# gau-nernst/vision-toolbox

Measured on AMD Instinct MI355X. Metric: images/sec (node) CSPDarknet-53 bf16 train step @224px, higher is better.
Workload: dtype bf16; 1 GPU; cspdarknet53 train step (fwd+CE+bwd+allreduce+SGD), batch 256/GPU, 3x224x224, 1000 classes, BASELINE configs[1]; global_batch=256, per_gpu_batch=256, parallelism=dp1, rccl_ranks=1, local_device=cuda:0, hip_graphs=False, main_stream_priority=-1, sync_bn=False, deterministic=False

## Files before the change

vision-toolbox_amd/csrc/vt_igemm.hip:

```cpp
#include <stdlib.h>

#include "vt_common.h"
#include "vt_igemm_args.h"

namespace {

constexpr int kTapBytes = VT_MAX_TAPS * 16;
constexpr int stat_bytes(int WM, int BN) { return WM * 2 * BN * 4 > 2048 ? WM * 2 * BN * 4 : 2048; }

__device__ __attribute__((aligned(16))) unsigned int vt_zero16[4];

__device__ __forceinline__ int swz(int row) { return (0x1320 >> (((row >> 2) & 3) * 4)) & 3; }

__device__ __forceinline__ void glds16(const void* gsrc, unsigned lds_base) {
    unsigned keep;
    asm volatile(
        "s_mov_b32 %0, m0\n\t"
        "s_mov_b32 m0, %2\n\t"
        "s_nop 0\n\t"
        "global_load_lds_dwordx4 %1, off\n\t"
        "s_mov_b32 m0, %0"
        : "=&s"(keep)
        : "v"(gsrc), "s"(lds_base)
        : "memory");
}

template <int N>
__device__ __forceinline__ void vm_wait() {
    asm volatile("s_waitcnt vmcnt(%0)" ::"n"(N) : "memory");
}

template <typename T>
__device__ __forceinline__ void mma(const uint4& a, const uint4& b, f32x4& acc);

template <>
__device__ __forceinline__ void mma<bf16_t>(const uint4& a, const uint4& b, f32x4& acc) {
    acc = __builtin_amdgcn_mfma_f32_16x16x32_bf16(__builtin_bit_cast(bf16x8, a),
                                                  __builtin_bit_cast(bf16x8, b), acc, 0, 0, 0);
}
template <>
__device__ __forceinline__ void mma<float>(const uint4& a, const uint4& b, f32x4& acc) {
    acc = __builtin_amdgcn_mfma_f32_16x16x4f32(__uint_as_float(a.x), __uint_as_float(b.x), acc, 0, 0, 0);
    acc = __builtin_amdgcn_mfma_f32_16x16x4f32(__uint_as_float(a.y), __uint_as_float(b.y), acc, 0, 0, 0);
    acc = __builtin_amdgcn_mfma_f32_16x16x4f32(__uint_as_float(a.z), __uint_as_float(b.z), acc, 0, 0, 0);
    acc = __builtin_amdgcn_mfma_f32_16x16x4f32(__uint_as_float(a.w), __uint_as_float(b.w), acc, 0, 0, 0);
}

template <int BM, int BN, int PD, int NW, int WM>
struct Geom {
    static constexpr int NI_A = BM / 16;
    static constexpr int NI = (BM + BN) / 16;
    static constexpr int IT = (NI + NW - 1) / NW;
    static constexpr int SS = IT * NW * 64;
    static constexpr int HDR = kTapBytes + stat_bytes(WM, BN);
    static constexpr int NS = PD + 1;
    static constexpr int STAGE_BYTES = NS * SS * 16;
};

template <typename T, int BM, int BN, int WM, int WN, int PD, bool UK>
__global__ void __launch_bounds__(64 * WM * WN) igemm_kernel(const IgemmArgs p) {
    constexpr int NW = WM * WN;
    using G = Geom<BM, BN, PD, NW, WM>;
    constexpr int NT = 64 * NW;
    constexpr int kHdrBytes = G::HDR;
    constexpr int EPC = 16 / sizeof(T);
    constexpr int BK = 4 * EPC;
    constexpr int TM = BM / WM, TN = BN / WN, FM = TM / 16, FN = TN / 16;
    constexpr int IT = G::IT, SS = G::SS, NS = G::NS;
    static_assert(NW == 4 || NW == 8, "4 or 8 waves per workgroup");
    static_assert(TM % 16 == 0 && TN % 16 == 0, "wave tile must be 16-granular");
    static_assert(BN <= 160, "filter tile width");
    static_assert(BM % 16 == 0 && BN % 16 == 0, "tile rows come in groups of 16 per DMA instruction");
    static_assert(PD >= 1 && PD <= 3, "prefetch distance");

    extern __shared__ __attribute__((aligned(16))) char smem[];
    int4* sTap = (int4*)smem;
    float* sStat = (float*)(smem + kTapBytes);
    uint4* sStage = (uint4*)(smem + kHdrBytes);
    T* sOut = (T*)(smem + kHdrBytes);

    const int tid = threadIdx.x;
    const int lane = tid & 63;
    const int wave = __builtin_amdgcn_readfirstlane(tid >> 6);
    const int wm = wave / WN, wn = wave % WN;

    const int bid = blockIdx.x;
    const int xcd = bid & 7, slot = bid >> 3;
    const int tn = slot % p.tiles_n;
    const int ml = slot / p.tiles_n;
    const int tm = xcd * p.chunk + ml;
    if (ml >= p.chunk || tm >= p.tiles_m) return;

#pragma unroll
    for (int t = 0; t < VT_MAX_TAPS; ++t) {
        if (t < p.ntaps && tid == t) {
            const int dh = p.dh[t], dw = p.dw[t];
            sTap[t] = make_int4(dh, dw, (dh * p.Wi + dw) * p.ldx, 0);
        }
    }
    if (tid < 2 * BN) sStat[tid] = 0.f;
    __syncthreads();

    const T* __restrict__ xg = (const T*)p.x;
    const T* __restrict__ wg = (const T*)p.w;
    const unsigned long zero_src = (unsigned long)(const void*)vt_zero16;
    const unsigned ring_base = (unsigned)(unsigned long)(__attribute__((address_space(3))) char*)sStage;

    const int cj = (lane & 3) ^ ((0x1320 >> (((lane >> 4) & 3) * 4)) & 3);
    int hb[IT], wb[IT];
    long off0[IT];
    bool valid[IT];
    const int HoWo = p.Ho * p.Wo;
#pragma unroll
    for (int i = 0; i < IT; ++i) {
        const int j = wave + NW * i;
        hb[i] = wb[i] = 0;
        off0[i] = 0;
        valid[i] = false;
        if (j < G::NI_A) {
            const int row = j * 16 + (lane >> 2);
            const int m = tm * BM + row;
            valid[i] = m < p.M;
            const int mm = valid[i] ? m : 0;
            const int b = mm / HoWo;
            const int rem = mm - b * HoWo;
            const int oi = rem / p.Wo;
            const int oj = rem - oi * p.Wo;
            hb[i] = oi * p.sh + p.h0;
            wb[i] = oj * p.sw + p.w0;
            off0[i] = ((long)(b * p.Hi + hb[i]) * p.Wi + wb[i]) * p.ldx;
        } else if (j < G::NI) {
            const int n = tn * BN + (j - G::NI_A) * 16 + (lane >> 2);
            valid[i] = n < p.Cout;
            off0[i] = (long)(valid[i] ? n : 0) * p.ldw;
        }
    }

    int kk = cj * EPC;
    int tap = kk / p.Cin;
    int c = kk - tap * p.Cin;

    unsigned long abase[IT], amask[IT], bptr[IT];
    unsigned bstep[IT];
    int tap_u = 0, c0_u = 0;
    if constexpr (UK) {
#pragma unroll
        for (int i = 0; i < IT; ++i) {
            const int j = wave + NW * i;
            abase[i] = (unsigned long)(xg + (off0[i] + cj * EPC));
            amask[i] = 0;
            bptr[i] = zero_src;
            bstep[i] = 0;
            if (j < G::NI_A) {
                if (valid[i]) {
                    for (int t = 0; t < p.ntaps; ++t) {
                        const int4 te = sTap[t];
                        if ((unsigned)(hb[i] + te.x) < (unsigned)p.Hi && (unsigned)(wb[i] + te.y) < (unsigned)p.Wi)
                            amask[i] |= 1ul << t;
                    }
                }
            } else if (j < G::NI && valid[i]) {
                bptr[i] = (unsigned long)(wg + (off0[i] + cj * EPC));
                bstep[i] = BK * (unsigned)sizeof(T);
            }
        }
    }

#define VT_ISSUE_STAGE(st)                                                                      \
    do {                                                                                        \
        if constexpr (UK) {                                                                     \
            const long koff = ((long)__builtin_amdgcn_readfirstlane(sTap[tap_u].z) + c0_u) * (long)sizeof(T); \
            _Pragma("unroll") for (int i = 0; i < IT; ++i) {                                    \
                const int j = wave + NW * i;                                                     \
                const bool isA = (NW * i + NW - 1 < G::NI_A) ? true : (NW * i >= G::NI_A ? false : j < G::NI_A); \
                unsigned long ps;                                                               \
                if (isA) {                                                                      \
                    ps = ((amask[i] >> tap_u) & 1ul) ? abase[i] + koff : zero_src;              \
                } else {                                                                        \
                    ps = bptr[i];                                                               \
                    bptr[i] += bstep[i];                                                        \
                }                                                                               \
                glds16((const void*)ps, ring_base + (unsigned)(((st)*SS + j * 64) * 16));       \
            }                                                                                   \
            c0_u += BK;                                                                         \
            if (c0_u >= p.Cin) {                                                                \
                c0_u = 0;                                                                       \
                ++tap_u;                                                                        \
            }                                                                                   \
            break;                                                                              \
        }                                                                                       \
        const bool kval = tap < p.ntaps;                                                        \
        const int4 te = sTap[kval ? tap : 0];                                                   \
        _Pragma("unroll") for (int i = 0; i < IT; ++i) {                                        \
            const int j = wave + NW * i;                                                         \
              \
            const bool isA = (NW * i + NW - 1 < G::NI_A) ? true : (NW * i >= G::NI_A ? false : j < G::NI_A); \
            const bool isB = !isA && ((NW * i + NW - 1 < G::NI) ? true : (NW * i >= G::NI ? false : j < G::NI)); \
            const bool va = kval && valid[i] && (unsigned)(hb[i] + te.x) < (unsigned)p.Hi &&    \
                            (unsigned)(wb[i] + te.y) < (unsigned)p.Wi;                          \
            const unsigned long pa = (unsigned long)(xg + (off0[i] + te.z + c));                \
            const unsigned long pb = (unsigned long)(wg + (off0[i] + kk));                      \
            const unsigned long ps = isA ? (va ? pa : zero_src) : ((isB && kval && valid[i]) ? pb : zero_src); \
            glds16((const void*)ps, ring_base + (unsigned)(((st)*SS + j * 64) * 16));           \
        }                                                                                       \
        kk += BK;                                                                               \
        c += BK;                                                                                \
        while (c >= p.Cin) {                                                                    \
            c -= p.Cin;                                                                         \
            ++tap;                                                                              \
        }                                                                                       \
    } while (0)

    f32x4 acc[FM][FN];
#pragma unroll
    for (int i = 0; i < FM; ++i)
#pragma unroll
        for (int j = 0; j < FN; ++j) acc[i][j] = f32x4{0.f, 0.f, 0.f, 0.f};

    const int lane_off = (lane & 15) * 4 + ((lane >> 4) ^ swz(lane & 15));
    const int nk = (p.Ktot + BK - 1) / BK;

#pragma unroll
    for (int s = 0; s < PD; ++s)
        if (s < nk) VT_ISSUE_STAGE(s);

    int cur = 0;
    int nxt = PD % NS;
    for (int ks = 0; ks < nk; ++ks) {
        const int younger = min(PD - 1, nk - 1 - ks);
        if (younger >= 2)
            vm_wait<2 * IT>();
        else if (younger == 1)
            vm_wait<IT>();
        else
            vm_wait<0>();
        __builtin_amdgcn_s_barrier();
        asm volatile("" ::: "memory");
        if (ks + PD < nk) VT_ISSUE_STAGE(nxt);
        {
            const uint4* A = sStage + cur * SS + wm * TM * 4 + lane_off;
            const uint4* Bt = sStage + cur * SS + BM * 4 + wn * TN * 4 + lane_off;
            uint4 af[FM], bf[FN];
#pragma unroll
            for (int i = 0; i < FM; ++i) af[i] = A[i * 64];
#pragma unroll
            for (int j = 0; j < FN; ++j) bf[j] = Bt[j * 64];
#if VT_MFMA_SETPRIO
            __builtin_amdgcn_s_setprio(1);
#endif
#pragma unroll
            for (int i = 0; i < FM; ++i)
#pragma unroll
                for (int j = 0; j < FN; ++j) mma<T>(af[i], bf[j], acc[i][j]);
#if VT_MFMA_SETPRIO
            __builtin_amdgcn_s_setprio(0);
#endif
        }
        cur = (cur + 1 == NS) ? 0 : cur + 1;
        nxt = (nxt + 1 == NS) ? 0 : nxt + 1;
    }
#undef VT_ISSUE_STAGE
    __syncthreads();

    const bool affine = p.flags & VT_CONV_AFFINE;
    const bool relu = p.flags & VT_CONV_RELU;
    const bool stats = p.flags & VT_CONV_STATS;
#pragma unroll
    for (int j = 0; j < FN; ++j) {
        const int col = wn * TN + j * 16 + (lane & 15);
        const int n = tn * BN + col;
        float sc = 1.f, sf = 0.f;
        if (affine && n < p.Cout) {
            if (p.scale) sc = p.scale[n];
            sf = p.shift[n];
        }
        float s = 0.f, ss = 0.f;
#pragma unroll
        for (int i = 0; i < FM; ++i) {
#pragma unroll
            for (int r = 0; r < 4; ++r) {
                float v = acc[i][j][r];
                if (affine) v = fmaf(v, sc, sf);
                if (relu) v = fmaxf(v, 0.f);
                const T tv = from_float<T>(v);
                const int row = wm * TM + i * 16 + (lane >> 4) * 4 + r;
                sOut[row * BN + col] = tv;
                const float fv = (float)tv;
                s += fv;
                ss += fv * fv;
            }
        }
        if (stats) {
            s += __shfl_xor(s, 16, 64);
            s += __shfl_xor(s, 32, 64);
            ss += __shfl_xor(ss, 16, 64);
            ss += __shfl_xor(ss, 32, 64);
            if (lane < 16) {
                sStat[(wm * 2 + 0) * BN + col] = s;
                sStat[(wm * 2 + 1) * BN + col] = ss;
            }
        }
    }
    __syncthreads();

    if (stats && tid < 2 * BN) {
        const int which = tid / BN, col = tid % BN;
        const int n = tn * BN + col;
        if (n < p.Cout) {
            float acc = 0.f;
#pragma unroll
            for (int w = 0; w < WM; ++w) acc += sStat[(w * 2 + which) * BN + col];
            vt_stat_add(p.stats, ((long)(tm % kStatReplicas) * 2 + which) * p.Cout + n, acc);
        }
    }

    constexpr int CPR = BN / EPC;
    const uint4* sOut4 = (const uint4*)sOut;
    T* __restrict__ yg = (T*)p.y;
    const T* __restrict__ rg = (const T*)p.res;
    const bool has_res = (p.flags & VT_CONV_RESIDUAL) != 0;
    auto out_pixel = [&](int m) -> long {
        if (p.dense_out) return m;
        const int b = m / HoWo;
        const int rem = m - b * HoWo;
        const int oi = rem / p.Wo;
        const int oj = rem - oi * p.Wo;
        return ((long)b * p.oH + (oi * p.oHs + p.oh0)) * p.oW + (oj * p.oWs + p.ow0);
    };
    if (has_res) {
        constexpr int ITER = (BM * CPR + NT - 1) / NT, RB = 4;
#pragma unroll
        for (int b0 = 0; b0 < ITER; b0 += RB) {
            uint4 rr[RB];
            long oy[RB];
            bool ok[RB];
#pragma unroll
            for (int u = 0; u < RB; ++u) {
                const int idx = tid + (b0 + u) * NT;
                const int row = idx / CPR, ch = idx % CPR;
                const int m = tm * BM + row;
                const int n = tn * BN + ch * EPC;
                ok[u] = b0 + u < ITER && idx < BM * CPR && m < p.M && n < p.Cout;
                const long po = ok[u] ? out_pixel(m) : 0;
                oy[u] = po * p.ldy + vt_out_col(p, n, p.ldy);
                rr[u] = *(const uint4*)(rg + (ok[u] ? po * p.ldr + vt_out_col(p, n, p.ldr) : 0l));
            }
#pragma unroll
            for (int u = 0; u < RB; ++u) {
                if (!ok[u]) continue;
                float fv[EPC], fr[EPC];
                VecIO<T>::unpack(sOut4[tid + (b0 + u) * NT], fv);
                VecIO<T>::unpack(rr[u], fr);
#pragma unroll
                for (int e = 0; e < EPC; ++e) fv[e] += fr[e];
                *(uint4*)(yg + oy[u]) = VecIO<T>::pack(fv);
            }
        }
        return;
    }
#pragma unroll 2
    for (int idx = tid; idx < BM * CPR; idx += NT) {
        const int row = idx / CPR, ch = idx % CPR;
        const int m = tm * BM + row;
        const int n = tn * BN + ch * EPC;
        if (m < p.M && n < p.Cout) *(uint4*)(yg + (out_pixel(m) * p.ldy + vt_out_col(p, n, p.ldy))) = sOut4[idx];
    }
}

template <typename T, int BM, int BN, int WM, int WN, int PD>
int launch(IgemmArgs& a, hipStream_t st) {
    using G = Geom<BM, BN, PD, WM * WN, WM>;
    constexpr int kHdrBytes = G::HDR;
    a.tiles_m = (a.M + BM - 1) / BM;
    a.tiles_n = (a.Cout + BN - 1) / BN;
    a.chunk = (a.tiles_m + 7) / 8;
    constexpr int outb = BM * BN * (int)sizeof(T);
    constexpr int smem = kHdrBytes + (G::STAGE_BYTES > outb ? G::STAGE_BYTES : outb);
    static_assert(smem <= 160 * 1024, "tile exceeds the 160 KiB LDS of a gfx950 CU");
    const long blocks = (long)8 * a.chunk * a.tiles_n;
    if (blocks > 0x7fffffffL) {
        vt_set_error("vt_conv_igemm: grid too large (%ld blocks)", blocks);
        return VT_ERR_UNSUPPORTED;
    }
    constexpr int BKe = 4 * (16 / (int)sizeof(T));
    auto kern = (a.Cin % BKe == 0) ? igemm_kernel<T, BM, BN, WM, WN, PD, true>
                                   : igemm_kernel<T, BM, BN, WM, WN, PD, false>;
    if (smem > 64 * 1024) {
        const int rc = vt_raise_dynamic_lds((const void*)kern, smem, "vt_conv_igemm");
        if (rc != VT_OK) return rc;
    }
    vt_note_kernel("igemm_kernel<%s,%d,%d,%d,%d,%d,uk%d>", sizeof(T) == 2 ? "bf16" : "f32", BM, BN, WM, WN, PD,
                   (int)(a.Cin % BKe == 0));
    hipLaunchKernelGGL(kern, dim3((unsigned)blocks), dim3(64 * WM * WN), smem, st, a);
    VT_CHECK_LAUNCH("vt_conv_igemm");
    return VT_OK;
}

}

static void fill_args(IgemmArgs& a, const vt_conv_desc* d, const void* x, const void* w, void* y, const float* scale,
                      const float* shift, const void* residual, float* stats) {
    memset(&a, 0, sizeof(a));
    a.x = x;
    a.w = w;
    a.y = y;
    a.scale = scale;
    a.shift = shift;
    a.res = residual;
    a.stats = stats;
    a.B = d->B, a.Hi = d->Hi, a.Wi = d->Wi, a.Cin = d->Cin, a.ldx = d->ldx;
    a.Ho = d->Ho, a.Wo = d->Wo, a.sh = d->sh, a.sw = d->sw, a.h0 = d->h0, a.w0 = d->w0;
    a.Cout = d->Cout, a.ldy = d->ldy, a.oH = d->oH, a.oW = d->oW;
    a.oHs = d->oHs, a.oWs = d->oWs, a.oh0 = d->oh0, a.ow0 = d->ow0;
    a.ldw = d->ldw, a.ldr = d->ldr, a.flags = d->flags, a.ntaps = d->ntaps;
    a.M = d->B * d->Ho * d->Wo;
    a.Ktot = d->ntaps * d->Cin;
    a.dense_out = (d->oHs == 1 && d->oWs == 1 && d->oh0 == 0 && d->ow0 == 0 && d->oH == d->Ho && d->oW == d->Wo);
    memcpy(a.dh, d->dh, VT_MAX_TAPS);
    memcpy(a.dw, d->dw, VT_MAX_TAPS);

}

extern "C" int vt_conv_igemm(const vt_conv_desc* d, const void* x, const void* w, void* y,
                             const float* scale, const float* shift, const void* residual,
                             float* stats, void* stream) {
    VT_REQUIRE(d && x && w && (y || (d->flags & VT_CONV_NOSTORE)), VT_ERR_INVALID, "vt_conv_igemm: null argument");
    VT_REQUIRE(!(d->flags & VT_CONV_NOSTORE) || (d->flags & VT_CONV_STATS), VT_ERR_INVALID,
               "vt_conv_igemm: NOSTORE is the statistics-only pass");
    VT_REQUIRE(d->dtype == VT_F32 || d->dtype == VT_BF16, VT_ERR_UNSUPPORTED,
               "vt_conv_igemm: dtype %d", d->dtype);
    VT_REQUIRE(!(d->flags & VT_CONV_BNRED), VT_ERR_INVALID, "vt_conv_igemm: unknown flag bits 0x%x", d->flags);
    const int epc = vt_epc(d->dtype);
    VT_REQUIRE(d->ntaps >= 1 && d->ntaps <= VT_MAX_TAPS, VT_ERR_UNSUPPORTED,
               "vt_conv_igemm: ntaps %d outside [1,%d]", d->ntaps, VT_MAX_TAPS);
    VT_REQUIRE(d->B > 0 && d->Hi > 0 && d->Wi > 0 && d->Ho > 0 && d->Wo > 0 && d->Cin > 0 && d->Cout > 0,
               VT_ERR_INVALID, "vt_conv_igemm: non-positive extent");
    VT_REQUIRE(d->Cin % epc == 0 && d->Cout % epc == 0 && d->ldx % epc == 0 && d->ldy % epc == 0 &&
                   d->ldw % epc == 0,
               VT_ERR_UNSUPPORTED,
               "vt_conv_igemm: Cin=%d Cout=%d ldx=%d ldy=%d ldw=%d must be multiples of %d", d->Cin,
               d->Cout, d->ldx, d->ldy, d->ldw, epc);
    const bool d2s = (d->flags & VT_CONV_D2S) != 0;
    if (d2s) {
        VT_REQUIRE(d->Cout % (4 * epc) == 0 && d->oHs == 2 && d->oWs == 2 && d->oh0 == 0 && d->ow0 == 0 &&
                       d->oH == 2 * d->Ho && d->oW == 2 * d->Wo &&
                       !(d->flags & (VT_CONV_STATS | VT_CONV_AFFINE | VT_CONV_RELU)),
                   VT_ERR_UNSUPPORTED, "vt_conv_igemm: D2S needs Cout = 4*C', a 2x2-strided output and a raw epilogue");
    }
    VT_REQUIRE(d->ldx >= d->Cin && d->ldy >= (d2s ? d->Cout / 4 : d->Cout) && d->ldw >= d->ntaps * d->Cin, VT_ERR_INVALID,
               "vt_conv_igemm: stride smaller than extent");
    VT_REQUIRE(vt_aligned16(x) && vt_aligned16(w) && vt_aligned16(y), VT_ERR_INVALID,
               "vt_conv_igemm: x/w/y must be 16-byte aligned");
    VT_REQUIRE(d->oHs >= 1 && d->oWs >= 1 && d->oh0 >= 0 && d->ow0 >= 0 &&
                   (d->Ho - 1) * d->oHs + d->oh0 < d->oH && (d->Wo - 1) * d->oWs + d->ow0 < d->oW,
               VT_ERR_INVALID, "vt_conv_igemm: output placement outside the %dx%d tensor", d->oH, d->oW);
    const long in_elems = (long)d->B * d->Hi * d->Wi * d->ldx;
    const long out_elems = (long)d->B * d->oH * d->oW * d->ldy;
    VT_REQUIRE(in_elems < 0x7fffffffL && out_elems < 0x7fffffffL && (long)d->B * d->Ho * d->Wo < 0x7fffffffL,
               VT_ERR_UNSUPPORTED, "vt_conv_igemm: tensor exceeds 2^31 elements");
    if (d->flags & VT_CONV_RESIDUAL) {
        VT_REQUIRE(residual && vt_aligned16(residual) && d->ldr % epc == 0 && d->ldr >= (d2s ? d->Cout / 4 : d->Cout),
                   VT_ERR_INVALID, "vt_conv_igemm: bad residual");
    }
    if (d->flags & VT_CONV_AFFINE) VT_REQUIRE(shift, VT_ERR_INVALID, "vt_conv_igemm: AFFINE needs shift");
    if (d->flags & VT_CONV_STATS) {
        VT_REQUIRE(stats, VT_ERR_INVALID, "vt_conv_igemm: STATS needs a stats buffer");
        VT_REQUIRE(!(d->flags & (VT_CONV_AFFINE | VT_CONV_RELU | VT_CONV_RESIDUAL)), VT_ERR_UNSUPPORTED,
                   "vt_conv_igemm: STATS is only defined on the raw conv output");
    }

    IgemmArgs a;
    fill_args(a, d, x, w, y, scale, shift, residual, stats);

    hipStream_t st = (hipStream_t)stream;
    if (!d2s) {
        const int rc = vt_stem_dispatch(a, d->dtype, stream);
        if (rc >= 0) return rc;
        const int rc6 = vt_stem6_dispatch(a, d->dtype, stream);
        if (rc6 >= 0) return rc6;
    }
    VT_REQUIRE(!(d->flags & VT_CONV_NOSTORE), VT_ERR_UNSUPPORTED, "vt_conv_igemm: NOSTORE outside the RGB stem kernel");
    if (!d2s) {
        const int rc = vt_span6_dispatch(a, d->dtype, stream);
        if (rc >= 0) return rc;
    }
    {
        const int rc = vt_pspan_dispatch(a, d->dtype, stream);
        if (rc >= 0) return rc;
    }
    {
        const int rc = vt_span_dispatch(a, d->dtype, stream);
        if (rc >= 0) return rc;
    }
    if (d->dtype == VT_BF16) {
        const int w8 = VT_KNOB("VT_IGEMM_W8", 3);
        if (VT_KNOB("VT_IGEMM_BN80", 1) && d->Cout % 80 == 0 && d->Cout <= 160) {
            if ((w8 & 1) && d->Cout == 160) return launch<bf16_t, 256, 160, 4, 2, 2>(a, st);
            return launch<bf16_t, 256, 80, 4, 1, 2>(a, st);
        }
        if (d->Cout > 64 && (w8 & 2) && ((long)(a.M + 255) / 256) * ((d->Cout + 127) / 128) >= ((w8 & 4) ? 0 : 256))
            return launch<bf16_t, 256, 128, 4, 2, 2>(a, st);
        if (d->Cout > 64) return launch<bf16_t, 128, 128, 2, 2, 2>(a, st);
        if (d->Cout > 32) return launch<bf16_t, 128, 64, 2, 2, 2>(a, st);
        return launch<bf16_t, 256, 32, 4, 1, 2>(a, st);
    }
    if (d->Cout > 32) return launch<float, 128, 64, 2, 2, 2>(a, st);
    return launch<float, 128, 32, 4, 1, 2>(a, st);
}

extern "C" int vt_conv_dgrad_bnred(const vt_conv_desc* d, const void* dz, const void* w, void* dy, const void* z, int32_t ldz,
                                   const float* scale, const float* shift, const float* mean, const float* invstd,
                                   int32_t relu, float* sums, void* stream) {
    VT_REQUIRE(d && dz && w && dy && z && scale && shift && mean && invstd && sums, VT_ERR_INVALID,
               "vt_conv_dgrad_bnred: null argument");
    VT_REQUIRE(relu == 0 || relu == 1, VT_ERR_UNSUPPORTED, "vt_conv_dgrad_bnred: activation code %d (none / ReLU only)", relu);
    VT_REQUIRE(d->flags == 0, VT_ERR_INVALID, "vt_conv_dgrad_bnred: the launch has a plain epilogue (flags 0x%x)", d->flags);
    const long M = (long)d->B * d->oH * d->oW;
    const bool whole = d->oHs == 1 && d->oWs == 1 && d->oh0 == 0 && d->ow0 == 0 && d->oH == d->Ho && d->oW == d->Wo;
    VT_REQUIRE(whole, VT_ERR_INVALID, "vt_conv_dgrad_bnred: the launch must produce every pixel of d(y)");
    const int epc = vt_epc(d->dtype);
    VT_REQUIRE(ldz % epc == 0 && ldz >= d->Cout && vt_aligned16(z), VT_ERR_INVALID, "vt_conv_dgrad_bnred: bad z");
    if (d->dtype == VT_BF16 && VT_KNOB("VT_DGRAD_BNRED", 1) && d->ntaps >= 1 && d->ntaps <= VT_MAX_TAPS && d->Cin % epc == 0 &&
        d->Cout % epc == 0 && d->ldx % epc == 0 && d->ldy % epc == 0 && d->ldw % epc == 0 && d->ldx >= d->Cin &&
        d->ldy >= d->Cout && d->ldw >= d->ntaps * d->Cin && vt_aligned16(dz) && vt_aligned16(w) && vt_aligned16(dy) &&
        (long)d->B * d->Hi * d->Wi * d->ldx < 0x7fffffffL && M * d->ldy < 0x7fffffffL && M * ldz < 0x7fffffffL) {
        IgemmArgs a;
        fill_args(a, d, dz, w, dy, scale, shift, z, sums);
        a.ldr = ldz;
        a.aux0 = mean, a.aux1 = invstd;
        a.flags = VT_CONV_BNRED | (relu ? VT_CONV_RELU : 0);
        const int rc = vt_span6_dispatch(a, d->dtype, stream);
        if (rc >= 0) return rc;
    }
    const int rc = vt_conv_igemm(d, dz, w, dy, nullptr, nullptr, nullptr, nullptr, stream);
    if (rc != VT_OK) return rc;
    return vt_bn_act_bwd_reduce(dy, d->ldy, z, ldz, scale, shift, mean, invstd, M, d->Cout, relu, d->dtype, sums, stream);
}
```

vision-toolbox_amd/csrc/vt_igemm_args.h:

```cpp
#pragma once
#include "vt_common.h"

#define VT_CONV_BNRED 0x1000

#ifndef VT_MFMA_SETPRIO
#define VT_MFMA_SETPRIO 0
#endif

struct IgemmArgs {
    const void* x;
    const void* w;
    void* y;
    const float* scale;
    const float* shift;
    const void* res;
    float* stats;
    int B, Hi, Wi, Cin, ldx, Ho, Wo, sh, sw, h0, w0, Cout, ldy, oH, oW, oHs, oWs, oh0, ow0;
    int ldw, ldr, flags, ntaps;
    int M, Ktot, tiles_m, tiles_n, chunk, dense_out;
    int fast_dma;
    int8_t dh[VT_MAX_TAPS];
    int8_t dw[VT_MAX_TAPS];
    const float* aux0;
    const float* aux1;
};

__device__ __forceinline__ long vt_out_col(const IgemmArgs& p, int n, int ld) {
    if (!(p.flags & VT_CONV_D2S)) return n;
    const int cq = p.Cout >> 2;
    const int blk = n / cq;
    return ((long)(blk >> 1) * p.oW + (blk & 1)) * ld + (n - blk * cq);
}

int vt_span_dispatch(IgemmArgs& a, int dtype, void* stream);

int vt_span6_dispatch(IgemmArgs& a, int dtype, void* stream);

int vt_pspan_dispatch(IgemmArgs& a, int dtype, void* stream);

int vt_stem_dispatch(IgemmArgs& a, int dtype, void* stream);

int vt_stem6_dispatch(IgemmArgs& a, int dtype, void* stream);
```

Baseline: 13220 images/sec.

## Add persistent weight-stationary 1x1 conv GEMM kernel with register ring prefetch

Adds a dedicated bf16 kernel for stride-1 1x1 convolutions. The kernel loads a full BN-column weight slab into LDS once per block. Waves then stream 32-row activation blocks through a 3–4 deep register ring feeding MFMA 16x16x32, with fused epilogue and optional fused BN statistics. It is dispatched ahead of the generic pspan/span paths, but only for a narrow M/Cin window, and by default only for the stats-producing case. The aim is to cut weight reloads and per-tile overhead of the generic implicit GEMM, at the cost of low occupancy and large LDS use.

```diff
diff --git a/vision-toolbox_amd/csrc/vt_gemm1x1.hip b/vision-toolbox_amd/csrc/vt_gemm1x1.hip
--- /dev/null
+++ b/vision-toolbox_amd/csrc/vt_gemm1x1.hip
@@ -0,0 +1,284 @@
+#include <type_traits>
+
+#include "vt_igemm_args.h"
+
+namespace {
+
+constexpr int kRows = 32;
+constexpr int kFM = kRows / 16;
+constexpr int kThreads = 512;
+
+struct G1Args {
+    IgemmArgs p;
+    int ksteps;
+    int nrb;
+    int gx, gy;
+};
+
+__device__ __forceinline__ float sum16(float x) {
+    x += __shfl_xor(x, 8, 64);
+    x += __shfl_xor(x, 4, 64);
+    x += __shfl_xor(x, 2, 64);
+    x += __shfl_xor(x, 1, 64);
+    return x;
+}
+
+template <int BN, bool STATS, int RS>
+__global__ __launch_bounds__(kThreads, 4) void gemm1x1_kernel(const G1Args a) {
+    constexpr int NF = BN / 16;
+    constexpr int NG = BN / 32;
+    extern __shared__ __attribute__((aligned(16))) char smem[];
+    const IgemmArgs& p = a.p;
+    const unsigned item = vt_xcd_item(blockIdx.x, gridDim.x, 8);
+    if (item >= (unsigned)(a.gx * a.gy)) return;
+    const int tn = (int)(item % (unsigned)a.gy), bx = (int)(item / (unsigned)a.gy);
+    const int n0 = tn * BN;
+    const int tid = threadIdx.x, lane = tid & 63;
+    const int wave = __builtin_amdgcn_readfirstlane(tid >> 6);
+    const int lrow = lane & 15, lq = lane >> 4;
+    const int KS = a.ksteps;
+
+    {
+        const bf16_t* __restrict__ wg = (const bf16_t*)p.w;
+        const int per_col = KS * 4;
+        for (int idx = tid; idx < BN * per_col; idx += kThreads) {
+            const int c = idx / per_col, rem = idx - c * per_col;
+            const int ks = rem >> 2, q4 = rem & 3;
+            uint4 v = make_uint4(0u, 0u, 0u, 0u);
+            if (n0 + c < p.Cout) v = *(const uint4*)(wg + ((long)(n0 + c) * p.ldw + ks * 32 + q4 * 8));
+            const int g = c >> 5, cc = c & 31;
+            const int f = 2 * g + ((cc >> 2) & 1), r = 4 * (cc >> 3) + (cc & 3);
+            *(uint4*)(smem + (((long)ks * NF + f) * 64 + (q4 * 16 + r)) * 16) = v;
+        }
+    }
+    __syncthreads();
+
+    const int stride = a.gx * (kThreads / 64);
+    const int first = bx * (kThreads / 64) + wave;
+    const bf16_t* __restrict__ xg = (const bf16_t*)p.x;
+    bf16_t* __restrict__ yg = (bf16_t*)p.y;
+    const bf16_t* rg = (const bf16_t*)p.res;
+    const bool has_res = (p.flags & VT_CONV_RESIDUAL) != 0;
+    const bool affine = (p.flags & VT_CONV_AFFINE) != 0;
+    const bool relu = (p.flags & VT_CONV_RELU) != 0;
+
+    float s1[STATS ? NG : 1][8], s2[STATS ? NG : 1][8];
+    if (STATS) {
+#pragma unroll
+        for (int g = 0; g < NG; ++g)
+#pragma unroll
+            for (int e = 0; e < 8; ++e) s1[g][e] = s2[g][e] = 0.f;
+    }
+
+    int rb_l = first, ks_l = 0;
+    const bf16_t* lp[kFM];
+    auto set_lp = [&]() __attribute__((always_inline)) {
+#pragma unroll
+        for (int i = 0; i < kFM; ++i) {
+            long m = (long)rb_l * kRows + i * 16 + lrow;
+            m = m < p.M ? m : (long)p.M - 1;
+            lp[i] = xg + (m * p.ldx + lq * 8);
+        }
+    };
+    set_lp();
+    uint4 ring[RS][kFM];
+#pragma unroll
+    for (int s = 0; s < RS; ++s)
+#pragma unroll
+        for (int i = 0; i < kFM; ++i) ring[s][i] = make_uint4(0u, 0u, 0u, 0u);
+    auto issue = [&](auto Sc) __attribute__((always_inline)) {
+        constexpr int S = decltype(Sc)::value;
+        if (rb_l < a.nrb) {
+#pragma unroll
+            for (int i = 0; i < kFM; ++i) ring[S][i] = *(const uint4*)(lp[i] + ks_l * 32);
+            if (++ks_l == KS) {
+                ks_l = 0;
+                rb_l += stride;
+                set_lp();
+            }
+        }
+    };
+
+    f32x4 acc[kFM][NF];
+    auto zero_acc = [&]() __attribute__((always_inline)) {
+#pragma unroll
+        for (int i = 0; i < kFM; ++i)
+#pragma unroll
+            for (int f = 0; f < NF; ++f) acc[i][f] = f32x4{0.f, 0.f, 0.f, 0.f};
+    };
+    zero_acc();
+
+    auto epilogue = [&](int rb) __attribute__((always_inline)) {
+#pragma unroll
+        for (int i = 0; i < kFM; ++i) {
+            const long m = (long)rb * kRows + i * 16 + lrow;
+            const bool row_ok = m < p.M;
+#pragma unroll
+            for (int g = 0; g < NG; ++g) {
+                const int ch = n0 + g * 32 + lq * 8;
+                const bool ok = row_ok && ch < p.Cout;
+                uint4 rr = make_uint4(0u, 0u, 0u, 0u);
+                if (!STATS && has_res && ok) rr = *(const uint4*)(rg + (m * p.ldr + ch));
+                float v[8];
+#pragma unroll
+                for (int e = 0; e < 8; ++e) v[e] = acc[i][2 * g + (e >> 2)][e & 3];
+                if (!STATS && (affine || relu) && ok) {
+#pragma unroll
+                    for (int e = 0; e < 8; ++e) {
+                        if (affine) v[e] = fmaf(v[e], p.scale ? p.scale[ch + e] : 1.f, p.shift[ch + e]);
+                        if (relu) v[e] = fmaxf(v[e], 0.f);
+                    }
+                }
+                uint4 out = VecIO<bf16_t>::pack(v);
+                if (ok) {
+                    if (STATS) {
+                        float r8[8];
+                        VecIO<bf16_t>::unpack(out, r8);
+#pragma unroll
+                        for (int e = 0; e < 8; ++e) {
+                            s1[g][e] += r8[e];
+                            s2[g][e] = fmaf(r8[e], r8[e], s2[g][e]);
+                        }
+                    }
+                    if (!STATS && has_res) {
+                        float fv[8], fr[8];
+                        VecIO<bf16_t>::unpack(out, fv);
+                        VecIO<bf16_t>::unpack(rr, fr);
+#pragma unroll
+                        for (int e = 0; e < 8; ++e) fv[e] += fr[e];
+                        out = VecIO<bf16_t>::pack(fv);
+                    }
+                    *(uint4*)(yg + (m * p.ldy + ch)) = out;
+                }
+            }
+        }
+    };
+
+    int rb = first, ks = 0;
+    const char* fl = smem + lane * 16;
+    auto step = [&](auto Sc) __attribute__((always_inline)) -> bool {
+        constexpr int S = decltype(Sc)::value;
+        if (rb >= a.nrb) return false;
+        issue(std::integral_constant<int, (S + RS - 1) % RS>{});
+        const char* fb = fl + (long)ks * (NF * 1024);
+#pragma unroll
+        for (int f0 = 0; f0 < NF; f0 += 4) {
+            uint4 bf[4];
+#pragma unroll
+            for (int f = 0; f < 4 && f0 + f < NF; ++f) bf[f] = *(const uint4*)(fb + (f0 + f) * 1024);
+#pragma unroll
+            for (int f = 0; f < 4 && f0 + f < NF; ++f)
+#pragma unroll
+                for (int i = 0; i < kFM; ++i)
+                    acc[i][f0 + f] = __builtin_amdgcn_mfma_f32_16x16x32_bf16(
+                        __builtin_bit_cast(bf16x8, bf[f]), __builtin_bit_cast(bf16x8, ring[S][i]), acc[i][f0 + f], 0, 0, 0);
+        }
+        if (++ks == KS) {
+            epilogue(rb);
+            zero_acc();
+            ks = 0;
+            rb += stride;
+        }
+        return true;
+    };
+    static_assert(RS == 3 || RS == 4, "the prologue and the trip below list their steps");
+    issue(std::integral_constant<int, 0>{});
+    issue(std::integral_constant<int, 1>{});
+    if constexpr (RS == 4) issue(std::integral_constant<int, 2>{});
+    for (;;) {
+        if (!step(std::integral_constant<int, 0>{})) break;
+        if (!step(std::integral_constant<int, 1>{})) break;
+        if (!step(std::integral_constant<int, 2>{})) break;
+        if constexpr (RS == 4) {
+            if (!step(std::integral_constant<int, 3>{})) break;
+        }
+    }
+
+    if (STATS) {
+        float* sFold = (float*)(smem + (long)KS * NF * 1024);
+#pragma unroll
+        for (int g = 0; g < NG; ++g)
+#pragma unroll
+            for (int e = 0; e < 8; ++e) {
+                const float u = sum16(s1[g][e]), v = sum16(s2[g][e]);
+                if (lrow == 0) {
+                    sFold[(wave * 2 + 0) * BN + g * 32 + lq * 8 + e] = u;
+                    sFold[(wave * 2 + 1) * BN + g * 32 + lq * 8 + e] = v;
+                }
+            }
+        __syncthreads();
+        const int rep = (int)(blockIdx.x % (unsigned)kStatReplicas);
+        for (int i = tid; i < 2 * BN; i += kThreads) {
+            const int which = i / BN, col = i - which * BN;
+            if (n0 + col < p.Cout) {
+                float t = 0.f;
+#pragma unroll
+                for (int w = 0; w < kThreads / 64; ++w) t += sFold[(w * 2 + which) * BN + col];
+                vt_stat_add(p.stats, ((long)rep * 2 + which) * p.Cout + n0 + col, t);
+            }
+        }
+    }
+}
+
+template <int BN, bool STATS, int RS>
+int g1_launch(G1Args& a, int occ, hipStream_t st) {
+    const IgemmArgs& p = a.p;
+    const int smem = a.ksteps * BN * 64 + (STATS ? (kThreads / 64) * 2 * BN * 4 : 0);
+    a.gy = (p.Cout + BN - 1) / BN;
+    const int waves = kThreads / 64;
+    long gx_max = (long)vt_device_cus() * occ / a.gy;
+    gx_max = gx_max < 1 ? 1 : gx_max;
+    const long per = (a.nrb + gx_max * waves - 1) / (gx_max * waves);
+    a.gx = (int)((a.nrb + per * waves - 1) / (per * waves));
+    auto kern = gemm1x1_kernel<BN, STATS, RS>;
+    if (smem > 64 * 1024) {
+        const int rc = vt_raise_dynamic_lds((const void*)kern, smem, "vt_conv_igemm(gemm1x1)");
+        if (rc != VT_OK) return rc;
+    }
+    vt_note_kernel("gemm1x1_kernel<bf16,%d,%s,occ%d>", BN, STATS ? "stats" : "plain", occ);
+    hipLaunchKernelGGL(kern, dim3(vt_xcd_grid((long)a.gx * a.gy)), dim3(kThreads), smem, st, a);
+    VT_CHECK_LAUNCH("vt_conv_igemm(gemm1x1)");
+    return VT_OK;
+}
+
+}
+
+int vt_gemm1x1_dispatch(IgemmArgs& a0, int dtype, void* stream) {
+    const int knob = VT_KNOB("VT_GEMM1X1", 1);
+    if (!knob || dtype != VT_BF16) return -1;
+    if (a0.flags & (VT_CONV_D2S | VT_CONV_NOSTORE | VT_CONV_BNRED)) return -1;
+    if (a0.ntaps != 1 || a0.sh != 1 || a0.sw != 1 || a0.Ho != a0.Hi || a0.Wo != a0.Wi || !a0.dense_out) return -1;
+    if (a0.h0 + a0.dh[0] != 0 || a0.w0 + a0.dw[0] != 0) return -1;
+    if (a0.Cin % 32 != 0 || a0.Cout % 8 != 0) return -1;
+    const bool stats = (a0.flags & VT_CONV_STATS) != 0;
+    if (stats && (a0.flags & (VT_CONV_AFFINE | VT_CONV_RELU | VT_CONV_RESIDUAL))) return -1;
+    if ((a0.flags & VT_CONV_RESIDUAL) && !a0.res) return -1;
+    const int ksteps = a0.Cin / 32;
+    int bn = (!stats && a0.Cout > 64) ? 128 : (a0.Cout > 32 ? 64 : 32);
+    while (bn > 32 && ksteps * bn * 64 > 64 * 1024) bn >>= 1;
+    if (ksteps * bn * 64 > 64 * 1024) return -1;
+    if (knob != 2) {
+        const int dirs = knob == 1 ? 4 : knob;
+        if (!(dirs & (stats ? 4 : 8))) return -1;
+        const long M = a0.M;
+        bool take = false;
+        if (a0.Cin <= 128) take = M >= 100352 && M <= 200704;
+        else if (a0.Cin <= 256) take = M > 100352 && M <= 200704 && (stats || a0.Cout <= 128);
+        if (!take) return -1;
+    }
+    G1Args a;
+    memset(&a, 0, sizeof(a));
+    a.p = a0;
+    a.ksteps = ksteps;
+    a.nrb = (a0.M + kRows - 1) / kRows;
+    int occ = VT_KNOB("VT_GEMM1X1_OCC", 0);
+    occ = occ < 1 ? (stats ? 1 : 2) : (occ > 2 ? 2 : occ);
+    hipStream_t st = (hipStream_t)stream;
+    if (stats) {
+        if (bn == 64) return g1_launch<64, true, 4>(a, occ, st);
+        return g1_launch<32, true, 4>(a, occ, st);
+    }
+    if (bn == 128) return g1_launch<128, false, 3>(a, occ, st);
+    if (bn == 64) return g1_launch<64, false, 4>(a, occ, st);
+    return g1_launch<32, false, 4>(a, occ, st);
+}
diff --git a/vision-toolbox_amd/csrc/vt_igemm.hip b/vision-toolbox_amd/csrc/vt_igemm.hip
--- a/vision-toolbox_amd/csrc/vt_igemm.hip
+++ b/vision-toolbox_amd/csrc/vt_igemm.hip
@@ -485,6 +485,10 @@
         if (rc >= 0) return rc;
     }
     {
+        const int rc = vt_gemm1x1_dispatch(a, d->dtype, stream);
+        if (rc >= 0) return rc;
+    }
+    {
         const int rc = vt_pspan_dispatch(a, d->dtype, stream);
         if (rc >= 0) return rc;
     }
diff --git a/vision-toolbox_amd/csrc/vt_igemm_args.h b/vision-toolbox_amd/csrc/vt_igemm_args.h
--- a/vision-toolbox_amd/csrc/vt_igemm_args.h
+++ b/vision-toolbox_amd/csrc/vt_igemm_args.h
@@ -38,6 +38,8 @@
 
 int vt_pspan_dispatch(IgemmArgs& a, int dtype, void* stream);
 
+int vt_gemm1x1_dispatch(IgemmArgs& a, int dtype, void* stream);
+
 int vt_stem_dispatch(IgemmArgs& a, int dtype, void* stream);
 
 int vt_stem6_dispatch(IgemmArgs& a, int dtype, void* stream);
```

New measurement: 13250 images/sec (median of 6 runs). About the same (+0.2%).
